# noway/nzcb-circom

Hardware: AMD Instinct MI355X
Metric: PLONK proofs/sec for nzcp_live (~2^21 constraints) at 1/2/4/8 MI355X (higher is better)
Workload: dtype u32 limbs: BN254 Fr/Fq Montgomery, 8x32-bit and 9x29-bit (MSM, NTT twiddles, quotient); 1 GPU; nzcp_live fullProve: NZCPPubIdentity(1,351,0,4,2,4) witness on the GPU (600560 signals) + PLONK proof, n=2^21, nPublic=3, 2970 inputs; domain_size=2097152, n_public=3, n_constraints=1785813, n_vars=1782570, n_additions=1182010, proofs_per_gpu=140, total_proofs=140, parallelism=batch-shard x1 (no collective), proofs_in_flight_per_gpu=5

## Files before the change

nzcb-circom_amd/csrc/prover.h:

```cpp
#pragma once
#include <chrono>
#include <functional>
#include <memory>
#include <string>
#include <vector>

#include "engine.h"
#include "zkey.h"

namespace nzcb {

struct AddRec {
  uint32_t ai, bi, dst, pad;
  Fr ac, bc;
};

struct MsmShard {
  static constexpr int kSlots = 3;
  int device = 0;
  size_t lo = 0, hi = 0;
  size_t llo = 0, lhi = 0;
  MsmBaseTable table, ltable;
  std::unique_ptr<MsmScratch> sc[kSlots];
  DevBuf<Fr> scal[kSlots];
  hipStream_t st[kSlots] = {nullptr, nullptr, nullptr};
  ~MsmShard();
};

struct Prover {
  uint32_t n = 0, n4 = 0, nVars = 0, nPublic = 0, nAdditions = 0, nConstraints = 0, nWit = 0;
  int power = 0;
  Fr k1, k2, wn, w2;
  std::vector<uint32_t> add_level_start;
  bool transcript_public = true;
  std::function<void(const std::string&)> log;

  std::unique_ptr<Engine> eng;
  static constexpr int kSlots = 3;
  std::unique_ptr<MsmScratch> msc[kSlots];
  hipStream_t aux[kSlots] = {nullptr, nullptr, nullptr};
  hipEvent_t ready[kSlots] = {nullptr, nullptr, nullptr};
  bool slot_split[kSlots] = {false, false, false};
  bool slot_lag[kSlots] = {false, false, false};
  hipEvent_t side_ready = nullptr, side_done = nullptr, pows_done = nullptr;
  ~Prover();
  DevBuf<G1Affine> ptau;
  MsmBaseTable ptab;
  DevBuf<G1Affine> ltau;
  MsmBaseTable ltab;
  bool lcommit = false;
  DevBuf<Fr> qm, ql, qr, qo, qc;
  DevBuf<Fr> sigma;
  DevBuf<Fr> sig_h;
  DevBuf<Fr> q_h;
  DevBuf<Fr> w_h;
  DevBuf<Fr> lagrange;
  DevBuf<uint32_t> amap, bmap, cmap;
  DevBuf<AddRec> adds;
  DevBuf<Fr> root_lo, root_hi;
  DevBuf<Fr> x_lo;
  DevBuf<Fr> g_lo, g_hi, gi_lo, gi_hi;
  DevBuf<F29> g29, gi29;
  Fr zh_inv[4];
  DevBuf<Fr> cq, cs, cl;
  bool quot3 = false;
  DevBuf<Fr> cq3, cs3, cl3;
  DevBuf<F29> tw3, itw3;
  Fr d3[3];
  Fr sig_top[3][4];
  DevBuf<Fr> wit;
  DevBuf<Fr> wtns_in;
  DevBuf<Fr> A, B, C, Z;
  DevBuf<Fr> pol_a, pol_b, pol_c, pol_z;
  DevBuf<Fr> A4, B4, C4, Z4, T, Tz, t;
  DevBuf<Fr> pol_r, pol_wxi, pol_wxiw;
  DevBuf<Fr> blind;
  DevBuf<Fr> scan_tmp;
  DevBuf<Fr> lin_tab;
  size_t lin_qn = 0;
  Fr* lin_tile_pows(int k);
  std::vector<Fr> lin_host;
  DevBuf<Fr> eval_part;
  DevBuf<F29> eval_pw;
  DevBuf<uint32_t> flags;
  std::vector<Fr> host_part;
  DevBuf<uint32_t> ntt_scr2;
  Fr* top_host = nullptr;
  static constexpr int kMbFlags = 24, kMbTotals = 25, kMbEvals = 27, kMbEvalMax = 8;
  size_t mb_apub = 0, mb_pubw = 0, mb_words = 0;

  int lane_id = 0;
  int fault = 0;
  double tm[11] = {0};
  bool prof_gpu = false;
  std::vector<std::pair<hipEvent_t, hipEvent_t>> span_ev;
  std::vector<int> span_kind;
  size_t spans_used = 0;
  size_t span_begin(int kind, hipStream_t s);
  void span_end(size_t i, hipStream_t s);
  void span_totals(double* msm_ms, double* ntt_ms);

  Prover(const uint8_t* zkey, size_t len, int device);
  Prover(const Prover& primary, int lane);
  void set_msm_devices(const std::vector<int>& devices);
  std::vector<std::unique_ptr<MsmShard>> shards;
  size_t own_hi = 0, own_lhi = 0;
  nzcb_msm_send_fn split_send = nullptr;
  nzcb_msm_gather_fn split_gather = nullptr;
  void* split_user = nullptr;
  int split_world = 1;
  size_t split_own = 0, split_own_l = 0;
  void set_msm_split(int world, size_t own_points, size_t own_lagrange, nzcb_msm_send_fn send,
                     nzcb_msm_gather_fn gather, void* user);
  void prove(const uint8_t* witness, size_t n_witness, const uint8_t* blinding, uint8_t* proof_out,
             uint8_t* pub_out, bool witness_on_device = false);

 private:
  hipStream_t st() const { return eng->stream; }
  void init_slots();
  void alloc_workspace();
  void to4t(const Fr* evals, Fr* coefs, Fr* evals4, const int* bidx, int nb, hipStream_t s = nullptr);
  void to4t_coefs(const Fr* evals, Fr* coefs, const int* bidx, int nb, hipStream_t s, uint32_t* scr = nullptr);
  void to4t_evals4(const Fr* coefs, Fr* evals4, int nb, hipStream_t s, uint32_t* scr = nullptr);
  void round3_quot3(const Fr& beta, const Fr& gamma, const Fr& alpha, hipStream_t s);
  void launch_gate_check(hipStream_t s);
  void copy_tops(hipStream_t s);
  void commit_start(int slot, const Fr* scalars, size_t len, const MsmBaseTable* tab = nullptr,
// ... 14 lines not shown
```

nzcb-circom_amd/csrc/prover.hip:

```cpp
#include <rocprofiler-sdk-roctx/roctx.h>
#include "lagrange.h"
#include "prover.h"
#include "transcript.h"

#include <cstring>
#include <cerrno>
#include <string>
#include <sys/random.h>

#include "keccak.h"

namespace nzcb {

static constexpr int kT = 256;
static constexpr uint32_t kZeroRef = 0xffffffffu;

__global__ void k_wit_to_mont(const Fr* __restrict__ in, Fr* __restrict__ out, size_t n) {
  size_t i = (size_t)blockIdx.x * blockDim.x + threadIdx.x;
  if (i >= n) return;
  out[i] = (i == 0) ? Fr::zero() : to_mont(in[i]);
}

__global__ void k_additions(const AddRec* __restrict__ recs, uint32_t count, Fr* __restrict__ wit) {
  uint32_t i = blockIdx.x * blockDim.x + threadIdx.x;
// ... 445 lines not shown
  for (int T = t1 - 1; T >= t0; T--) {
    suf = suf + h[T] * Q[T];
    h[T] = suf * Qinv[T];
  }
  if (tid == 0) h[m] = Fr::zero();
}

__global__ void k_stride4(const Fr* __restrict__ src, size_t n, Fr* __restrict__ dst) {
  const size_t i = (size_t)blockIdx.x * blockDim.x + threadIdx.x;
  if (i < n) dst[i] = src[4 * i];
}

struct QArgs {
  Fr beta, gamma, alpha, alpha2, bk1, bk2;
  Fr zhinv[4];
};

__global__ void __launch_bounds__(kT)
k_quotient_coset(const Fr* __restrict__ A, const Fr* __restrict__ B, const Fr* __restrict__ C,
                 const Fr* __restrict__ Z, const Fr* __restrict__ cq, const Fr* __restrict__ cs,
                 const Fr* __restrict__ cl, uint32_t npub, const Fr* __restrict__ Apub, size_t n,
                 const Fr* __restrict__ xlo, const Fr* __restrict__ xhi, QArgs q, Fr* __restrict__ T) {
  const size_t n4 = 4 * n;
  size_t i = (size_t)blockIdx.x * blockDim.x + threadIdx.x;
  if (i >= n4) return;
  const Fr a = A[i], b = B[i], c = C[i];
  const Fr x = xlo[i & 4095] * xhi[i >> 12];
  Fr gate = a * b * cq[i] + a * cq[n4 + i] + b * cq[2 * n4 + i] + c * cq[3 * n4 + i] + cq[4 * n4 + i];
  for (uint32_t j = 0; j < npub; j++) gate = gate - cl[j * n4 + i] * Apub[j];
  const Fr z = Z[i];
  const Fr bx = q.beta * x;
  Fr num = (a + bx + q.gamma) * (b + q.bk1 * x + q.gamma);
  num = num * (c + q.bk2 * x + q.gamma) * z;
  Fr den = (a + q.beta * cs[i] + q.gamma) * (b + q.beta * cs[n4 + i] + q.gamma);
  den = den * (c + q.beta * cs[2 * n4 + i] + q.gamma) * Z[(i + 4) & (n4 - 1)];
  const Fr e4 = (z - Fr::one()) * cl[i] * q.alpha2;
  T[i] = (gate + q.alpha * (num - den) + e4) * q.zhinv[i & 3];
}

constexpr uint32_t kQ29MaxPub = 8;

static bool quot3_enabled() {
  static const bool on = [] {
    const char* e = std::getenv("NZCB_QUOT3");
    return !(e && e[0] == '0');
  }();
  return on;
}
struct QArgs29 {
  F29 beta, bk1, bk2, alpha2, zhinv[4];
  F29 gamma, negone;
  int k23;
  F29 alpha;
};

template <int K>
__device__ __forceinline__ F29 q29_pi_chunk(const Fr* __restrict__ cl, const Fr* __restrict__ Apub, uint32_t j0,
                                            size_t n4, size_t i) {
  F29 pa[K], pb[K];
#pragma unroll
  for (int k = 0; k < K; k++) {
    pa[k] = split29(cl[(size_t)(j0 + k) * n4 + i]);
    pb[k] = split29(neg(Apub[j0 + k]));
  }
  return mulsum29<Fr29, K>(pa, pb);
}

__device__ __forceinline__ F29 q29_pi(const Fr* __restrict__ cl, const Fr* __restrict__ Apub, uint32_t j0,
                                      uint32_t cnt, size_t n4, size_t i) {
  switch (cnt) {
    case 1: return q29_pi_chunk<1>(cl, Apub, j0, n4, i);
    case 2: return q29_pi_chunk<2>(cl, Apub, j0, n4, i);
    case 3: return q29_pi_chunk<3>(cl, Apub, j0, n4, i);
    default: return q29_pi_chunk<4>(cl, Apub, j0, n4, i);
  }
}

template <bool THREE>
__global__ void __launch_bounds__(kT) __attribute__((amdgpu_waves_per_eu(4, 8)))
k_quotient_coset29(const Fr* __restrict__ A, const Fr* __restrict__ B, const Fr* __restrict__ C,
                   const Fr* __restrict__ Z, const Fr* __restrict__ cq, const Fr* __restrict__ cs,
                   const Fr* __restrict__ cl, uint32_t npub, const Fr* __restrict__ Apub, size_t n,
                   const Fr* __restrict__ xlo, const Fr* __restrict__ xhi, QArgs29 q, Fr* __restrict__ T) {
  const size_t n4 = (THREE ? 3 : 4) * n;
  size_t i = (size_t)blockIdx.x * blockDim.x + threadIdx.x;
  if (i >= n4) return;
  size_t ix, izw;
  int cj;
  if (THREE) {
    const int lg = __ffsll((long long)n) - 1;
    const size_t j = i >> lg, m = i & (n - 1);
    ix = 4 * m + j;
    izw = j * n + ((m + 1) & (n - 1));
    cj = (int)j;
  } else {
    ix = i;
    izw = (i + 4) & (n4 - 1);
    cj = (int)(i & 3);
  }
  const F29 a = split29(A[i]), b = split29(B[i]), c = split29(C[i]), z = split29(Z[i]);
  F29 gate;
  {
    const F29 ga[4] = {mul29<Fr29>(a, b), a, b, c};
    const F29 gb[4] = {split29(cq[i]), split29(cq[n4 + i]), split29(cq[2 * n4 + i]), split29(cq[3 * n4 + i])};
    gate = add29(mulsum29<Fr29, 4>(ga, gb), split29(cq[4 * n4 + i]));
  }
  if (npub > 0) gate = add29(gate, q29_pi(cl, Apub, 0, npub < 4 ? npub : 4, n4, i));
  if (npub > 4) gate = add29(gate, q29_pi(cl, Apub, 4, npub - 4, n4, i));
  const F29 x = mul29<Fr29>(split29(xlo[ix & 4095]), split29(xhi[ix >> 12]));
  const F29 bx = mul29<Fr29>(q.beta, x);
  const F29 bx2 = q.k23 ? add29(bx, bx) : mul29<Fr29>(q.bk1, x);
  const F29 bx3 = q.k23 ? add29(bx2, bx) : mul29<Fr29>(q.bk2, x);
  const F29 f1 = add29(add29(a, bx), q.gamma);
  const F29 f2 = add29(add29(b, bx2), q.gamma);
  const F29 f3 = add29(add29(c, bx3), q.gamma);
  const F29 num = mul29<Fr29>(mul29<Fr29>(mul29<Fr29>(f1, f2), f3), z);
  const F29 g1 = add29(add29(a, mul29<Fr29>(q.beta, split29(cs[i]))), q.gamma);
  const F29 g2 = add29(add29(b, mul29<Fr29>(q.beta, split29(cs[n4 + i]))), q.gamma);
  const F29 g3 = add29(add29(c, mul29<Fr29>(q.beta, split29(cs[2 * n4 + i]))), q.gamma);
  const F29 den = mul29<Fr29>(mul29<Fr29>(mul29<Fr29>(g1, g2), g3), split29(Z[izw]));
  const F29 pa[2] = {q.alpha, q.alpha2};
  const F29 pb[2] = {sub29(num, den, Fr29::K2), mul29<Fr29>(add29(z, q.negone), split29(cl[i]))};
  const F29 S = add29(gate, mulsum29<Fr29, 2>(pa, pb));
  T[i] = join_fr29(mul29<Fr29>(S, q.zhinv[cj]));
}

__global__ void __launch_bounds__(kT)
k_gate_h(const Fr* __restrict__ A, const Fr* __restrict__ B, const Fr* __restrict__ C, const Fr* __restrict__ qh,
         size_t n, uint32_t npub, uint32_t* __restrict__ flags) {
  const size_t m = (size_t)blockIdx.x * blockDim.x + threadIdx.x;
  if (m >= n) return;
  const Fr a = A[m], b = B[m], c = C[m];
  Fr g = qh[m] * a * b + qh[n + m] * a + qh[2 * n + m] * b + qh[3 * n + m] * c + qh[4 * n + m];
  if (m < npub) g = g - a;
  if (!g.is_zero()) atomicOr(flags, 1u);
}

struct T3Args {
  Fr c0[6], c1[6], c2[6], q3[6];
  Fr i4, two_over_d, inv_d2;
};
__global__ void __launch_bounds__(kT)
k_t_combine(const Fr* __restrict__ V, size_t n, T3Args a, Fr* __restrict__ t) {
  const size_t k = (size_t)blockIdx.x * blockDim.x + threadIdx.x;
  if (k >= n) return;
  Fr v0 = V[k], v1 = V[n + k], v2 = V[2 * n + k];
  if (k < 6) {
    v0 = v0 - a.c0[k];
    v1 = v1 - a.c1[k];
    v2 = v2 - a.c2[k];
  }
  const Fr sm = v0 + v2, dl = v0 - v2, im = dl * a.i4, v12 = v1 + v1;
  t[k] = sm + v12 - im;
  t[n + k] = dl * a.two_over_d;
  t[2 * n + k] = (sm - v12 + im) * a.inv_d2;
  if (k < 6) t[3 * n + k] = a.q3[k];
}

__global__ void k_root_n(Fr* __restrict__ out, const Fr* __restrict__ rlo, const Fr* __restrict__ rhi, size_t n) {
  const size_t i = (size_t)blockIdx.x * blockDim.x + threadIdx.x;
  if (i < n) out[i] = root4(rlo, rhi, 4 * i);
}

__global__ void k_fault_bump(Fr* x) {
  if (threadIdx.x == 0) x[0] = x[0] + Fr::one();
}

__global__ void k_dbl_pow(Fr* __restrict__ x, size_t m, int e) {
  size_t i = (size_t)blockIdx.x * blockDim.x + threadIdx.x;
  if (i >= m) return;
  Fr v = x[i];
  for (int k = 0; k < e; k++) v = v + v;
  x[i] = v;
}

static F29 f29_exp(Fr v, int extra) {
  for (int k = 0; k < extra; k++) v = v + v;
  return split29(v);
}

static constexpr int kEvalMax = 8;
static constexpr int kEvalBits = 16;
struct EvalSet {
  const Fr* p[kEvalMax];
  uint64_t len[kEvalMax];
  Fr x[kEvalMax];
  Fr x4096[kEvalMax];
  F29 x29[kEvalMax];
// ... 39 lines not shown
}

template <int NP>
__global__ void __launch_bounds__(kT) k_eval_multi(EvalSet es, const F29* __restrict__ pw, const Fr* __restrict__ pw2,
                                                   Fr* __restrict__ partial, int nblocks) {
  static_assert(NP <= kEvalMax && kEvalMax <= 4 * (kT / 64), "one 16-lane group per point");
  __shared__ Fr sh[kT / 64];
  __shared__ Fr bpow[kEvalMax];
  __shared__ Fr bsum[kEvalMax];
  {
    const int l = (int)(threadIdx.x & 63), k = l & 15, j = 4 * (int)(threadIdx.x >> 6) + (l >> 4);
    Fr f = Fr::one();
    if (j < NP && k < es.nbits && ((blockIdx.x >> k) & 1u)) f = pw2[j * kEvalBits + k];
    for (int m = 8; m >= 1; m >>= 1) f = f * shfl_fr(f, l ^ m);
    if (j < NP && k == 0) bpow[j] = f;
  }
  const size_t s = (size_t)blockIdx.x * kT * kEvalChunk2 + threadIdx.x;
  F29 acc[NP];
#pragma unroll
  for (int j = 0; j < NP; j++)
#pragma unroll
    for (int l = 0; l < 9; l++) acc[j].v[l] = 0;
  for (int m = kEvalChunk2 - 1; m >= 0; m--) {
    const size_t i = s + (size_t)m * kT;
#pragma unroll
    for (int j = 0; j < NP; j++)
      if (i < es.len[j]) {
        const F29 t = mul29<Fr29>(acc[j], es.y29[j]), c = split29(es.p[j][i]);
#pragma unroll
        for (int l = 0; l < 9; l++) acc[j].v[l] = t.v[l] + c.v[l];
      }
  }
#pragma unroll
  for (int j = 0; j < NP; j++) {
    const Fr r = block_sum_fr(join_fr29(mul29<Fr29>(acc[j], pw[(size_t)j * kT + threadIdx.x])), sh);
    if (threadIdx.x == 0) bsum[j] = r;
  }
  if (threadIdx.x < NP) partial[(size_t)threadIdx.x * nblocks + blockIdx.x] = bsum[threadIdx.x] * bpow[threadIdx.x];
}

__global__ void __launch_bounds__(kT) k_eval_sum(const Fr* __restrict__ partial, int nblocks, Fr* __restrict__ out) {
  __shared__ Fr sh[kT / 64];
  const int j = blockIdx.x;
  Fr acc = Fr::zero();
  for (int b = (int)threadIdx.x; b < nblocks; b += kT) acc = acc + partial[(size_t)j * nblocks + b];
  const Fr r = block_sum_fr(acc, sh);
  if (threadIdx.x == 0) {
    host_put(out + j, r);
    host_put_done();
  }
}

struct RArgs {
  Fr coefz, coef_ab, ea, eb, ec, coefs3;
};

__global__ void k_pol_r(const Fr* __restrict__ pz, const Fr* __restrict__ qm, const Fr* __restrict__ ql,
                        const Fr* __restrict__ qr, const Fr* __restrict__ qo, const Fr* __restrict__ qc,
                        const Fr* __restrict__ s3, size_t n, RArgs r, Fr* __restrict__ out) {
  size_t i = (size_t)blockIdx.x * blockDim.x + threadIdx.x;
  if (i >= n + 3) return;
  Fr v = r.coefz * pz[i];
  if (i < n) {
    v = v + r.coef_ab * qm[i] + r.ea * ql[i] + r.eb * qr[i] + r.ec * qo[i] + qc[i];
    v = v - r.coefs3 * s3[i];
  }
  out[i] = v;
}

struct WArgs {
  Fr xim, xi2m, v[7], w0sub;
};

__global__ void k_pol_wxi(const Fr* __restrict__ t, const Fr* __restrict__ pr, const Fr* __restrict__ pa,
                          const Fr* __restrict__ pb, const Fr* __restrict__ pc, const Fr* __restrict__ s1,
                          const Fr* __restrict__ s2, size_t n, WArgs wa, Fr* __restrict__ out) {
  size_t i = (size_t)blockIdx.x * blockDim.x + threadIdx.x;
  if (i >= n + 6) return;
  Fr w = wa.xi2m * t[2 * n + i];
  if (i < n) w = w + wa.xim * t[n + i] + t[i];
  if (i < n + 3) w = w + wa.v[1] * pr[i];
  if (i < n + 2) w = w + wa.v[2] * pa[i] + wa.v[3] * pb[i] + wa.v[4] * pc[i];
  if (i < n) w = w + wa.v[5] * s1[i] + wa.v[6] * s2[i];
  if (i == 0) w = w - wa.w0sub;
  out[i] = w;
}

__global__ void k_div_check(const Fr* __restrict__ src, Fr p0_adjust, const Fr* __restrict__ q, Fr d,
                            uint32_t* flags, uint32_t bit, uint32_t* __restrict__ mb_flags) {
  if (threadIdx.x || blockIdx.x) return;
  Fr p0 = src[0] - p0_adjust;
  if (!(p0 + d * q[0]).is_zero()) atomicOr(flags, bit);
  host_put(mb_flags, *flags);
  host_put_done();
}

__global__ void k_root_table(Fr* __restrict__ out, Fr base, Fr scale, size_t count) {
  size_t i = (size_t)blockIdx.x * blockDim.x + threadIdx.x;
  if (i >= count) return;
  out[i] = scale * pow_u64(base, i);
}

__global__ void k_factor29_table(F29* __restrict__ out, const Fr* __restrict__ lo, const Fr* __restrict__ hi, Fr scale,
                                 size_t count) {
  size_t i = (size_t)blockIdx.x * blockDim.x + threadIdx.x;
  if (i >= count) return;
  Fr v = lo[i & 4095] * hi[i >> 12] * scale;
#pragma unroll
  for (int k = 0; k < 5; k++) v = v + v;
  out[i] = split29(v);
}

static std::string fr_dec(const Fr& m) {
  Fr x = from_mont(m);
  uint32_t v[8];
  std::memcpy(v, x.v, 32);
  std::string s;
  bool nz = true;
  while (nz) {
    uint64_t rem = 0;
    nz = false;
    for (int i = 7; i >= 0; i--) {
      uint64_t cur = (rem << 32) | v[i];
      v[i] = (uint32_t)(cur / 10);
      rem = cur % 10;
      if (v[i]) nz = true;
    }
    s.push_back((char)('0' + rem));
  }
  return std::string(s.rbegin(), s.rend());
}

static Fr fr_small(uint64_t k) {
  Fr x = Fr::zero();
  x.v[0] = (uint32_t)k;
  x.v[1] = (uint32_t)(k >> 32);
  return to_mont(x);
}
// ... 233 lines not shown
                         q_h.p + (size_t)k * n);
    NZ_HIP(hipGetLastError());
  }
  if (quot3) {
    const size_t nhi3 = (n + 4095) / 4096;
    tw3.alloc((size_t)3 * n);
    itw3.alloc((size_t)3 * n);
    const Fr inv4n = inverse(fr_small(n4));
    DevBuf<Fr> lo, hi;
    for (int j = 0; j < 3; j++) {
      const Fr cj = g * pow_u64(w4, (uint64_t)j), cji = inverse(cj);
      d3[j] = pow_u64(cj, n);
      table(lo, nlo, cj, one);
      table(hi, nhi3, pow_u64(cj, 4096), one);
      hipLaunchKernelGGL(k_factor29_table, dim3(grid_for(n, kT, 1u << 30)), dim3(kT), 0, s, tw3.p + (size_t)j * n,
                         lo.p, hi.p, one, (size_t)n);
      NZ_HIP(hipStreamSynchronize(s));
      table(lo, nlo, cji, one);
      table(hi, nhi3, pow_u64(cji, 4096), one);
      hipLaunchKernelGGL(k_factor29_table, dim3(grid_for(n, kT, 1u << 30)), dim3(kT), 0, s, itw3.p + (size_t)j * n,
                         lo.p, hi.p, inv4n, (size_t)n);
      NZ_HIP(hipGetLastError());
      NZ_HIP(hipStreamSynchronize(s));
    }
    for (int k = 0; k < 3; k++)
      NZ_HIP(hipMemcpy(sig_top[k], sigma.p + (size_t)k * 5 * n + (n - 4), 4 * sizeof(Fr), hipMemcpyDeviceToHost));
  }
  if (quot3) {
    const uint32_t nl = nPublic > 0 ? nPublic : 1;
    const size_t n3 = (size_t)3 * n;
    cq3.alloc(5 * n3);
    cs3.alloc(3 * n3);
    cl3.alloc(nl * n3);
    auto coset3 = [&](const Fr* coefs, Fr* out) {
      for (int j = 0; j < 3; j++) {
        NttIo io;
        io.in_len = n;
        io.in_f = tw3.p + (size_t)j * n;
        ntt(eng->ntt_tables, coefs, out + (size_t)j * n, power, false, s, nullptr, &io);
      }
    };
    const DevBuf<Fr>* qs[5] = {&qm, &ql, &qr, &qo, &qc};
    for (int k = 0; k < 5; k++) coset3(qs[k]->p, cq3.p + (size_t)k * n3);
    for (int k = 0; k < 3; k++) coset3(sigma.p + (size_t)k * 5 * n, cs3.p + (size_t)k * n3);
    for (uint32_t j = 0; j < nl; j++) coset3(lagrange.p + (size_t)j * 5 * n, cl3.p + (size_t)j * n3);
    NZ_HIP(hipGetLastError());
    auto scale = [&](Fr* p, size_t m, int e) {
      hipLaunchKernelGGL(k_dbl_pow, dim3(grid_for(m, kT, 1u << 30)), dim3(kT), 0, s, p, m, e);
    };
    scale(cq3.p, n3, 10);
    scale(cq3.p + n3, 3 * n3, 5);
    scale(cl3.p, (size_t)nl * n3, 5);
    scale(x_lo.p, nlo, 5);
    NZ_HIP(hipGetLastError());
  } else {
    const uint32_t nl = nPublic > 0 ? nPublic : 1;
    cq.alloc((size_t)5 * n4);
    cs.alloc((size_t)3 * n4);
    cl.alloc((size_t)nl * n4);
    auto coset_eval = [&](const Fr* coefs, Fr* out) {
      NttIo io;
      io.in_len = n;
      io.in_f = g29.p;
      ntt(eng->ntt_tables, coefs, out, power + 2, false, s, nullptr, &io);
    };
    const DevBuf<Fr>* qs[5] = {&qm, &ql, &qr, &qo, &qc};
    for (int k = 0; k < 5; k++) coset_eval(qs[k]->p, cq.p + (size_t)k * n4);
    for (int k = 0; k < 3; k++) coset_eval(sigma.p + (size_t)k * 5 * n, cs.p + (size_t)k * n4);
    for (uint32_t j = 0; j < nl; j++) coset_eval(lagrange.p + (size_t)j * 5 * n, cl.p + (size_t)j * n4);
    NZ_HIP(hipGetLastError());
    if (nPublic <= kQ29MaxPub) {
      auto scale = [&](Fr* p, size_t m, int e) {
        hipLaunchKernelGGL(k_dbl_pow, dim3(grid_for(m, kT, 1u << 30)), dim3(kT), 0, s, p, m, e);
      };
      scale(cq.p, n4, 10);
      scale(cq.p + n4, 3 * n4, 5);
      scale(cl.p, (size_t)nl * n4, 5);
      scale(x_lo.p, nlo, 5);
      NZ_HIP(hipGetLastError());
    }
  }
  NZ_HIP(hipStreamSynchronize(s));
}

void Prover::init_slots() {
  for (int i = 0; i < kSlots; i++) {
    msc[i].reset(new MsmScratch());
#ifdef NZCB_AB_GENERIC
    msc[i]->init((size_t)n + 6, true, i == 0 ? 3 : 1, true);
#else
    msc[i]->init((size_t)n + 6, true, i == 0 ? 3 : 1, false);
#endif
    NZ_HIP(hipStreamCreateWithFlags(&aux[i], hipStreamNonBlocking));
    NZ_HIP(hipEventCreateWithFlags(&ready[i], hipEventDisableTiming));
  }
  NZ_HIP(hipEventCreateWithFlags(&side_ready, hipEventDisableTiming));
  NZ_HIP(hipEventCreateWithFlags(&side_done, hipEventDisableTiming));
  NZ_HIP(hipEventCreateWithFlags(&pows_done, hipEventDisableTiming));
  mb_apub = kMbEvals + kMbEvalMax;
  mb_pubw = mb_apub + nPublic;
  mb_words = mb_pubw + nPublic;
  NZ_HIP(hipHostMalloc((void**)&top_host, mb_words * sizeof(Fr), hipHostMallocCoherent));
  std::memset((void*)top_host, 0, mb_words * sizeof(Fr));
}

void Prover::alloc_workspace() {
  wit.alloc(nVars ? nVars : 1);
  wtns_in.alloc(nWit ? nWit : 1);
  A.alloc(n + 2); B.alloc(n + 2); C.alloc(n + 2); Z.alloc(n);
  pol_a.alloc(n + 2); pol_b.alloc(n + 2); pol_c.alloc(n + 2); pol_z.alloc(n + 3);
  const size_t ne = quot3 ? (size_t)3 * n : n4;
  A4.alloc(ne); B4.alloc(ne); C4.alloc(ne); Z4.alloc(ne);
  T.alloc(ne); Tz.alloc(ne); t.alloc(quot3 ? ne + 6 : n4);
  pol_r.alloc(n + 3); pol_wxi.alloc(n + 6); pol_wxiw.alloc(n + 3);
  blind.alloc(13);
  scan_tmp.alloc(3 * ((size_t)n / kTileN + 2) + 64);
  lin_qn = (size_t)n / kTileN + 3;
  lin_tab.alloc(2 * sizeof(LinTab) / sizeof(Fr) + 4 * lin_qn);
  lin_host.resize(2 * sizeof(LinTab) / sizeof(Fr));
  size_t nblocks = ((size_t)3 * n + 6 + (size_t)kT * kEvalChunk2 - 1) / ((size_t)kT * kEvalChunk2) + 1;
  eval_part.alloc((size_t)kEvalMax * nblocks + kEvalMax);
  eval_pw.alloc((size_t)kEvalMax * kT + (kEvalMax * kEvalBits * sizeof(Fr) + sizeof(F29) - 1) / sizeof(F29));
  host_part.resize(std::max<size_t>(nblocks, kEvalMax));
  flags.p = (uint32_t*)(blind.p + 12);
  flags.n = 1;
  flags.owned = false;
  const int zlog = quot3 ? power : power + 2;
  if (zlog > 8) ntt_scr2.alloc((size_t)9 << zlog);
}

Prover::Prover(const Prover& pk, int lane) {
  GuardScope guards;
  lane_id = lane;
  n = pk.n; n4 = pk.n4; nVars = pk.nVars; nPublic = pk.nPublic; nAdditions = pk.nAdditions;
  nConstraints = pk.nConstraints; nWit = pk.nWit; power = pk.power;
  k1 = pk.k1; k2 = pk.k2; wn = pk.wn; w2 = pk.w2;
  add_level_start = pk.add_level_start;
  transcript_public = pk.transcript_public;
  for (int k = 0; k < 4; k++) zh_inv[k] = pk.zh_inv[k];
  NZ_HIP(hipSetDevice(pk.eng->device));
  eng.reset(new Engine(pk.eng->device, power + 2, 0));
  init_slots();
  ptau.alias(pk.ptau);
  ptab.q.alias(pk.ptab.q);
  ptab.n = pk.ptab.n; ptab.stride = pk.ptab.stride; ptab.c = pk.ptab.c; ptab.nw = pk.ptab.nw;
  ptab.mont_folded = pk.ptab.mont_folded;
  lcommit = pk.lcommit;
  ltau.alias(pk.ltau);
  ltab.q.alias(pk.ltab.q);
  ltab.n = pk.ltab.n; ltab.stride = pk.ltab.stride; ltab.c = pk.ltab.c; ltab.nw = pk.ltab.nw;
  ltab.sparse = pk.ltab.sparse;
  qm.alias(pk.qm); ql.alias(pk.ql); qr.alias(pk.qr); qo.alias(pk.qo); qc.alias(pk.qc);
  sigma.alias(pk.sigma); sig_h.alias(pk.sig_h); q_h.alias(pk.q_h); w_h.alias(pk.w_h); lagrange.alias(pk.lagrange);
  amap.alias(pk.amap); bmap.alias(pk.bmap); cmap.alias(pk.cmap); adds.alias(pk.adds);
  root_lo.alias(pk.root_lo); root_hi.alias(pk.root_hi); x_lo.alias(pk.x_lo);
  g_lo.alias(pk.g_lo); g_hi.alias(pk.g_hi); gi_lo.alias(pk.gi_lo); gi_hi.alias(pk.gi_hi);
  g29.alias(pk.g29); gi29.alias(pk.gi29);
  cq.alias(pk.cq); cs.alias(pk.cs); cl.alias(pk.cl);
  quot3 = pk.quot3;
  cq3.alias(pk.cq3); cs3.alias(pk.cs3); cl3.alias(pk.cl3);
  tw3.alias(pk.tw3); itw3.alias(pk.itw3);
  for (int j = 0; j < 3; j++) d3[j] = pk.d3[j];
  std::memcpy(sig_top, pk.sig_top, sizeof(sig_top));
  alloc_workspace();
}

void Prover::launch_gate_check(hipStream_t s) {
  hipLaunchKernelGGL(k_gate_h, dim3(grid_for(n, kT, 1u << 30)), dim3(kT), 0, s, A.p, B.p, C.p, q_h.p, (size_t)n,
                     nPublic, flags.p);
  NZ_HIP(hipGetLastError());
}

void Prover::copy_tops(hipStream_t s) {
  hipLaunchKernelGGL(k_tops, dim3(1), dim3(32), 0, s, pol_a.p, pol_b.p, pol_c.p, pol_z.p, (size_t)n,
                     (const uint32_t*)flags.p, top_host);
  NZ_HIP(hipGetLastError());
  NZ_HIP(hipStreamSynchronize(s));
  if (top_host[kMbFlags].v[0] & 1u) throw Error(NZCB_ERR_T_DIV, "T Polynomial is not divisible");
}

void Prover::round3_quot3(const Fr& beta, const Fr& gamma, const Fr& alpha, hipStream_t s) {
  const size_t n3 = (size_t)3 * n;
  const bool side = lcommit;
  if (side) copy_tops(s);
  QArgs29 q29;
  q29.beta = f29_exp(beta, 5);
  q29.k23 = k1 == fr_small(2) && k2 == fr_small(3) ? 1 : 0;
  q29.bk1 = f29_exp(beta * k1, 5);
  q29.bk2 = f29_exp(beta * k2, 5);
  q29.alpha2 = f29_exp(alpha * alpha, 5);
  for (int k = 0; k < 4; k++) q29.zhinv[k] = f29_exp(zh_inv[k], 5);
  q29.gamma = f29_exp(gamma, 0);
  q29.negone = f29_exp(neg(Fr::one()), 0);
  q29.alpha = f29_exp(alpha, 20);
  hipLaunchKernelGGL((k_quotient_coset29<true>), dim3(grid_for(n3, kT, 1u << 30)), dim3(kT), 0, s, A4.p, B4.p, C4.p,
                     Z4.p, cq3.p, cs3.p, cl3.p, nPublic, A.p, (size_t)n, x_lo.p, root_hi.p, q29, T.p);
  if (!side) launch_gate_check(s);
  for (int j = 0; j < 3; j++) {
    NttIo io;
    io.out_f = itw3.p + (size_t)j * n;
    io.out_f_has_scale = true;
    {
      const size_t sp = prof_gpu ? span_begin(1, s) : 0;
      ntt(eng->ntt_tables, T.p + (size_t)j * n, Tz.p + (size_t)j * n, power, true, s, nullptr, &io);
      if (prof_gpu) span_end(sp, s);
    }
  }
  NZ_HIP(hipGetLastError());
  if (!side) copy_tops(s);
  Fr top[4][6];
  std::memcpy(top, top_host, sizeof(top));
  Fr p1[4][6], p2[4][6];
  const Fr w = wn, wi = inverse(wn);
  const Fr wpow[6] = {w * w, w, Fr::one(), wi, wi * wi, wi * wi * wi};
  for (int u = 0; u < 6; u++) {
    for (int f3 = 0; f3 < 3; f3++) {
      p1[f3][u] = top[f3][5 - u];
      p2[f3][u] = top[f3][5 - u];
      if (u >= 2) p2[f3][u] = p2[f3][u] + beta * sig_top[f3][5 - u];
    }
    p1[3][u] = top[3][5 - u];
    p2[3][u] = top[3][5 - u] * wpow[u];
  }
  auto conv = [](const Fr (&x)[6], const Fr (&y)[6], Fr (&out)[6]) {
    for (int s2 = 0; s2 < 6; s2++) {
      Fr acc = Fr::zero();
      for (int u = 0; u <= s2; u++) acc = acc + x[u] * y[s2 - u];
      out[s2] = acc;
    }
  };
  Fr e1[6], e2[6], e3[6], h1[6], h2[6], h3[6];
  conv(p1[0], p1[1], e1);
  conv(e1, p1[2], e2);
  conv(e2, p1[3], e3);
  conv(p2[0], p2[1], h1);
  conv(h1, p2[2], h2);
  conv(h2, p2[3], h3);
  T3Args ta;
  const Fr D = d3[0], D3 = D * D * D, i4 = d3[1] * inverse(D), quarter = inverse(fr_small(4));
  for (int k = 0; k < 6; k++) {
    ta.q3[k] = alpha * (e3[5 - k] - h3[5 - k]);
    const Fr c = D3 * ta.q3[k] * quarter;
    ta.c0[k] = c;
    ta.c1[k] = neg(i4 * c);
    ta.c2[k] = neg(c);
  }
  ta.i4 = i4;
  ta.two_over_d = fr_small(2) * inverse(D);
  ta.inv_d2 = inverse(D * D);
// ... 455 lines not shown
    hipLaunchKernelGGL(k_perm_tile, dim3((unsigned)ntiles), dim3(kT), 0, s, A.p, B.p, C.p, sig_h.p, (size_t)n,
                       w_h.p, pa, Z.p, ntot, dtot);
    hipLaunchKernelGGL(k_perm_factors, dim3(1), dim3(1024), 0, s, (const Fr*)ntot, (const Fr*)dtot, (int)ntiles,
                       fac, top_host + kMbTotals);
    NZ_HIP(hipGetLastError());
    NZ_HIP(hipStreamSynchronize(s));
    const Fr tt[2] = {top_host[kMbTotals], top_host[kMbTotals + 1]};
    if (tt[0] != tt[1]) throw Error(NZCB_ERR_COPY, "Copy constraints does not match");
    hipLaunchKernelGGL(k_apply_tiles, dim3((unsigned)ntiles), dim3(kT), 0, s, Z.p, (size_t)n,
                       (const Fr*)fac, inverse(tt[1]));
    NZ_HIP(hipGetLastError());
    const int bz[3] = {9, 8, 7};
    to4t_coefs(Z.p, pol_z.p, bz, 3, s, ntt_scr2.p);
    lg("multiexp Z");
    commit_start(0, pol_z.p, n + 3);
    to4t_evals4(pol_z.p, Z4.p, 3, s, ntt_scr2.p);
    pZ = commit_finish(0);
  }
  tm[3] = ms_since(t2);

  ranges.next("round3: quotient t + commit T1, T2, T3");
  auto t3 = std::chrono::steady_clock::now();
  Fr alpha;
  {
    std::vector<uint8_t> tr(64);
    g1_uncompressed(pZ, tr.data());
    alpha = hash_to_fr(tr);
    lg("alpha: " + fr_dec(alpha));
  }
  {
    QArgs q;
    q.beta = beta;
    q.gamma = gamma;
    q.alpha = alpha;
    q.alpha2 = alpha * alpha;
    q.bk1 = beta * k1;
    q.bk2 = beta * k2;
    for (int k = 0; k < 4; k++) q.zhinv[k] = zh_inv[k];
    auto tq = std::chrono::steady_clock::now();
    NZ_HIP(hipStreamWaitEvent(s, side_done, 0));
    if (quot3) {
      round3_quot3(beta, gamma, alpha, s);
    } else if (nPublic <= kQ29MaxPub) {
      QArgs29 q29;
      q29.beta = f29_exp(beta, 5);
      q29.k23 = k1 == fr_small(2) && k2 == fr_small(3) ? 1 : 0;
      q29.bk1 = f29_exp(q.bk1, 5);
      q29.bk2 = f29_exp(q.bk2, 5);
      q29.alpha2 = f29_exp(q.alpha2, 5);
      for (int k = 0; k < 4; k++) q29.zhinv[k] = f29_exp(zh_inv[k], 5);
      q29.gamma = f29_exp(gamma, 0);
      q29.negone = f29_exp(neg(Fr::one()), 0);
      q29.alpha = f29_exp(alpha, 20);
      hipLaunchKernelGGL((k_quotient_coset29<false>), dim3(grid_for(n4, kT, 1u << 30)), dim3(kT), 0, s, A4.p, B4.p,
                         C4.p, Z4.p, cq.p, cs.p, cl.p, nPublic, A.p, (size_t)n, x_lo.p, root_hi.p, q29, T.p);
    } else {
      hipLaunchKernelGGL(k_quotient_coset, dim3(grid_for(n4, kT, 1u << 30)), dim3(kT), 0, s, A4.p, B4.p, C4.p,
                         Z4.p, cq.p, cs.p, cl.p, nPublic, A.p, (size_t)n, x_lo.p, root_hi.p, q, T.p);
    }
    NZ_HIP(hipGetLastError());
    if (!quot3) {
      NttIo io;
      io.out_f = gi29.p;
      io.out_f_has_scale = true;
      io.out_limit = (size_t)3 * n + 6;
      io.out_flags = flags.p;
      {
        const size_t sp = prof_gpu ? span_begin(1, s) : 0;
        ntt(eng->ntt_tables, T.p, t.p, power + 2, true, s, nullptr, &io);
        if (prof_gpu) span_end(sp, s);
      }
      NZ_HIP(hipGetLastError());
      uint32_t f = 0;
      NZ_HIP(hipMemcpyAsync(&f, flags.p, 4, hipMemcpyDeviceToHost, s));
      NZ_HIP(hipStreamSynchronize(s));
      if (f & 1u) throw Error(NZCB_ERR_T_DIV, "T Polynomial is not divisible");
    }
    ntt_ms += ms_since(tq);
    if (fault == NZCB_FAULT_QUOTIENT) {
      fault = 0;
      hipLaunchKernelGGL(k_fault_bump, dim3(1), dim3(64), 0, s, t.p + 1);
      NZ_HIP(hipGetLastError());
    }
    lg("multiexp T1");
    commit_start(0, t.p, n);
    lg("multiexp T2");
    commit_start(1, t.p + n, n);
    lg("multiexp T3");
    commit_start(2, t.p + 2 * (size_t)n, n + 6);
    pT1 = commit_finish(0);
    pT2 = commit_finish(1);
    pT3 = commit_finish(2);
  }
  tm[4] = ms_since(t3);

  ranges.next("round4: evaluations");
  auto t4 = std::chrono::steady_clock::now();
  Fr xi, ea, eb, ec, es1, es2, et, ezw, er, xim;
  {
    std::vector<uint8_t> tr(192);
    g1_uncompressed(pT1, tr.data());
    g1_uncompressed(pT2, tr.data() + 64);
    g1_uncompressed(pT3, tr.data() + 128);
    xi = hash_to_fr(tr);
    lg("xi: " + fr_dec(xi));
    {
      const Fr* polys[7] = {pol_a.p, pol_b.p, pol_c.p, sigma.p, sigma.p + 5 * (size_t)n, t.p, pol_z.p};
      const size_t lens[7] = {n + 2, n + 2, n + 2, n, n, 3 * (size_t)n + 6, n + 3};
      const Fr xs[7] = {xi, xi, xi, xi, xi, xi, xi * wn};
      Fr ev[7];
      eval_many(7, polys, lens, xs, ev, [&] {
        lin_tables(0, xi, aux[2]);
        lin_tables(1, xi * wn, aux[2]);
        NZ_HIP(hipEventRecord(pows_done, aux[2]));
      });
      NZ_HIP(hipStreamWaitEvent(s, pows_done, 0));
      ea = ev[0];
      eb = ev[1];
      ec = ev[2];
      es1 = ev[3];
      es2 = ev[4];
      et = ev[5];
      ezw = ev[6];
    }
    Fr coef_ab = ea * eb;
    Fr betaxi = beta * xi;
    Fr e2 = (ea + betaxi + gamma) * (eb + betaxi * k1 + gamma);
    e2 = e2 * (ec + betaxi * k2 + gamma) * alpha;
    Fr e3 = (ea + beta * es1 + gamma) * (eb + beta * es2 + gamma);
    e3 = e3 * beta * ezw * alpha;
    xim = xi;
    for (int i = 0; i < power; i++) xim = sqr(xim);
    Fr eval_l1 = (xim - Fr::one()) * inverse((xi - Fr::one()) * fr_small(n));
    Fr e4 = eval_l1 * (alpha * alpha);
    RArgs ra{e2 + e4, coef_ab, ea, eb, ec, e3};
    hipLaunchKernelGGL(k_pol_r, dim3(grid_for(n + 3, kT, 1u << 30)), dim3(kT), 0, s, pol_z.p, qm.p, ql.p, qr.p,
                       qo.p, qc.p, sigma.p + 10 * (size_t)n, (size_t)n, ra, pol_r.p);
    NZ_HIP(hipGetLastError());
    {
      const Fr* polys[1] = {pol_r.p};
      const size_t lens[1] = {n + 3};
      eval_many(1, polys, lens, &xi, &er);
    }
    {
      const Fr zh = xim - Fr::one(), nf = fr_small(n);
      Fr pi = Fr::zero(), wj = Fr::one();
      for (uint32_t j = 0; j < nPublic; j++) {
        pi = pi - Apub[j] * wj * zh * inverse(nf * (xi - wj));
        wj = wj * wn;
      }
      const Fr perm = alpha * (ea + beta * es1 + gamma) * (eb + beta * es2 + gamma) * (ec + gamma) * ezw;
      if (et * zh != er + pi - perm - e4)
        throw Error(NZCB_ERR_INTERNAL, "quotient check failed: t(xi) Z_H(xi) differs from the numerator at xi");
    }
  }
  tm[5] = ms_since(t4);

  ranges.next("round5: Wxi, Wxiw + commit");
  auto t5 = std::chrono::steady_clock::now();
  {
    std::vector<uint8_t> tr(7 * 32);
    const Fr* ev[7] = {&ea, &eb, &ec, &es1, &es2, &ezw, &er};
    for (int i = 0; i < 7; i++) fr_to_be(*ev[i], tr.data() + 32 * i);
    WArgs wa;
    wa.v[0] = Fr::zero();
    wa.v[1] = hash_to_fr(tr);
    lg("v: " + fr_dec(wa.v[1]));
    for (int i = 2; i <= 6; i++) wa.v[i] = wa.v[i - 1] * wa.v[1];
    wa.xim = xim;
    wa.xi2m = xim * xim;
    wa.w0sub = et + wa.v[1] * er + wa.v[2] * ea + wa.v[3] * eb + wa.v[4] * ec + wa.v[5] * es1 + wa.v[6] * es2;
    hipLaunchKernelGGL(k_pol_wxi, dim3(grid_for(n + 6, kT, 1u << 30)), dim3(kT), 0, s, t.p, pol_r.p, pol_a.p,
                       pol_b.p, pol_c.p, sigma.p, sigma.p + 5 * (size_t)n, (size_t)n, wa, T.p);
    NZ_HIP(hipGetLastError());
    div_pol1(T.p, n + 6, 0, Fr::zero(), pol_wxi.p, 4u);
    lg("multiexp Wxi");
    commit_start(0, pol_wxi.p, n + 6);
    div_pol1(pol_z.p, n + 3, 1, ezw, pol_wxiw.p, 4u);
    lg("multiexp Wxiw");
    commit_start(1, pol_wxiw.p, n + 3);
    NZ_HIP(hipStreamSynchronize(s));
    const uint32_t f = top_host[kMbFlags].v[0];
    pWxi = commit_finish(0);
    pWxiw = commit_finish(1);
    if (f & 4u) throw Error(NZCB_ERR_DIVPOL, "Polinomial does not divide");
  }
  tm[6] = ms_since(t5);
  tm[0] = ms_since(T0);
  tm[7] = msm_ms;
  tm[8] = ntt_ms;
  tm[9] = tm[10] = -1;
  if (prof_gpu) span_totals(&tm[9], &tm[10]);

  const G1Affine* pts[9] = {&pA, &pB, &pC, &pZ, &pT1, &pT2, &pT3, &pWxi, &pWxiw};
  for (int i = 0; i < 9; i++) {
    uint8_t* o = proof_out + 64 * i;
    if (pts[i]->is_inf()) {
      std::memset(o, 0, 64);
    } else {
      Fq x = from_mont(pts[i]->x), y = from_mont(pts[i]->y);
      std::memcpy(o, x.v, 32);
      std::memcpy(o + 32, y.v, 32);
    }
  }
  const Fr* ev[7] = {&ea, &eb, &ec, &es1, &es2, &ezw, &er};
  for (int i = 0; i < 7; i++) fr_to_le_normal(*ev[i], proof_out + 9 * 64 + 32 * i);
  for (uint32_t i = 0; i < nPublic; i++) {
    fr_to_le_normal(top_host[mb_pubw + i], pub_out + 32 * (size_t)i);
  }
}

}
```

Before: 47.49 proofs/s.

## Port pol_r, pol_wxi and gate check to 29-bit limbs; fold coset scaling

Rewrites k_pol_r, k_pol_wxi and the gate check kernel to use the 9x29-bit lazy-reduction arithmetic with mulsum dot products instead of serial 8x32 Montgomery ops. In the 3-coset quotient path it precomputes beta*x_hi per block and folds the per-coset Z_H inverse into the selector and Lagrange tables and into alpha. This removes one multiply per element in the quotient kernel and the final zhinv multiply. It adds setup-time table rescaling and depends on the lazy-reduction exponent bounds in f29_exp being correct.

```diff
diff --git a/nzcb-circom_amd/csrc/prover.h b/nzcb-circom_amd/csrc/prover.h
--- a/nzcb-circom_amd/csrc/prover.h
+++ b/nzcb-circom_amd/csrc/prover.h
@@ -73,6 +73,7 @@
   DevBuf<Fr> A, B, C, Z;
   DevBuf<Fr> pol_a, pol_b, pol_c, pol_z;
   DevBuf<Fr> A4, B4, C4, Z4, T, Tz, t;
+  DevBuf<Fr> bx_hi;
   DevBuf<Fr> pol_r, pol_wxi, pol_wxiw;
   DevBuf<Fr> blind;
   DevBuf<Fr> scan_tmp;
diff --git a/nzcb-circom_amd/csrc/prover.hip b/nzcb-circom_amd/csrc/prover.hip
--- a/nzcb-circom_amd/csrc/prover.hip
+++ b/nzcb-circom_amd/csrc/prover.hip
@@ -521,7 +521,22 @@
   F29 gamma, negone;
   int k23;
   F29 alpha;
+  F29 alphaz[3];
 };
+
+__global__ void k_beta_xhi(const Fr* __restrict__ xhi, Fr beta, size_t count, Fr* __restrict__ bxhi) {
+  const size_t k = (size_t)blockIdx.x * blockDim.x + threadIdx.x;
+  if (k < count) bxhi[k] = beta * xhi[k];
+}
+
+struct Z3Args {
+  Fr z[3];
+};
+__global__ void k_scale_coset3(Fr* __restrict__ p, size_t n, size_t arrays, Z3Args za) {
+  const size_t i = (size_t)blockIdx.x * blockDim.x + threadIdx.x;
+  if (i >= arrays * 3 * n) return;
+  p[i] = p[i] * za.z[(i / n) % 3];
+}
 
 template <int K>
 __device__ __forceinline__ F29 q29_pi_chunk(const Fr* __restrict__ cl, const Fr* __restrict__ Apub, uint32_t j0,
@@ -550,7 +565,8 @@
 k_quotient_coset29(const Fr* __restrict__ A, const Fr* __restrict__ B, const Fr* __restrict__ C,
                    const Fr* __restrict__ Z, const Fr* __restrict__ cq, const Fr* __restrict__ cs,
                    const Fr* __restrict__ cl, uint32_t npub, const Fr* __restrict__ Apub, size_t n,
-                   const Fr* __restrict__ xlo, const Fr* __restrict__ xhi, QArgs29 q, Fr* __restrict__ T) {
+                   const Fr* __restrict__ xlo, const Fr* __restrict__ xhi, const Fr* __restrict__ bxhi, QArgs29 q,
+                   Fr* __restrict__ T) {
   const size_t n4 = (THREE ? 3 : 4) * n;
   size_t i = (size_t)blockIdx.x * blockDim.x + threadIdx.x;
   if (i >= n4) return;
@@ -576,10 +592,17 @@
   }
   if (npub > 0) gate = add29(gate, q29_pi(cl, Apub, 0, npub < 4 ? npub : 4, n4, i));
   if (npub > 4) gate = add29(gate, q29_pi(cl, Apub, 4, npub - 4, n4, i));
-  const F29 x = mul29<Fr29>(split29(xlo[ix & 4095]), split29(xhi[ix >> 12]));
-  const F29 bx = mul29<Fr29>(q.beta, x);
-  const F29 bx2 = q.k23 ? add29(bx, bx) : mul29<Fr29>(q.bk1, x);
-  const F29 bx3 = q.k23 ? add29(bx2, bx) : mul29<Fr29>(q.bk2, x);
+  F29 bx, bx2, bx3;
+  if (THREE && q.k23) {
+    bx = mul29<Fr29>(split29(bxhi[ix >> 12]), split29(xlo[ix & 4095]));
+    bx2 = add29(bx, bx);
+    bx3 = add29(bx2, bx);
+  } else {
+    const F29 x = mul29<Fr29>(split29(xlo[ix & 4095]), split29(xhi[ix >> 12]));
+    bx = mul29<Fr29>(q.beta, x);
+    bx2 = q.k23 ? add29(bx, bx) : mul29<Fr29>(q.bk1, x);
+    bx3 = q.k23 ? add29(bx2, bx) : mul29<Fr29>(q.bk2, x);
+  }
   const F29 f1 = add29(add29(a, bx), q.gamma);
   const F29 f2 = add29(add29(b, bx2), q.gamma);
   const F29 f3 = add29(add29(c, bx3), q.gamma);
@@ -588,10 +611,13 @@
   const F29 g2 = add29(add29(b, mul29<Fr29>(q.beta, split29(cs[n4 + i]))), q.gamma);
   const F29 g3 = add29(add29(c, mul29<Fr29>(q.beta, split29(cs[2 * n4 + i]))), q.gamma);
   const F29 den = mul29<Fr29>(mul29<Fr29>(mul29<Fr29>(g1, g2), g3), split29(Z[izw]));
-  const F29 pa[2] = {q.alpha, q.alpha2};
+  const F29 pa[2] = {THREE ? q.alphaz[cj] : q.alpha, q.alpha2};
   const F29 pb[2] = {sub29(num, den, Fr29::K2), mul29<Fr29>(add29(z, q.negone), split29(cl[i]))};
   const F29 S = add29(gate, mulsum29<Fr29, 2>(pa, pb));
-  T[i] = join_fr29(mul29<Fr29>(S, q.zhinv[cj]));
+  if constexpr (THREE)
+    T[i] = canon_fr29(S);
+  else
+    T[i] = join_fr29(mul29<Fr29>(S, q.zhinv[cj]));
 }
 
 __global__ void __launch_bounds__(kT)
@@ -599,10 +625,12 @@
          size_t n, uint32_t npub, uint32_t* __restrict__ flags) {
   const size_t m = (size_t)blockIdx.x * blockDim.x + threadIdx.x;
   if (m >= n) return;
-  const Fr a = A[m], b = B[m], c = C[m];
-  Fr g = qh[m] * a * b + qh[n + m] * a + qh[2 * n + m] * b + qh[3 * n + m] * c + qh[4 * n + m];
-  if (m < npub) g = g - a;
-  if (!g.is_zero()) atomicOr(flags, 1u);
+  const F29 a = split29(A[m]), b = split29(B[m]), c = split29(C[m]);
+  const F29 ga[4] = {mul29<Fr29>(a, b), a, b, c};
+  const F29 gb[4] = {split29(qh[m]), split29(qh[n + m]), split29(qh[2 * n + m]), split29(qh[3 * n + m])};
+  F29 g = add29(mulsum29<Fr29, 4>(ga, gb), split29(qh[4 * n + m]));
+  if (m < npub) g = sub29(g, a, Fr29::K2);
+  if (!canon_fr29(g).is_zero()) atomicOr(flags, 1u);
 }
 
 struct T3Args {
@@ -748,38 +776,56 @@
 }
 
 struct RArgs {
-  Fr coefz, coef_ab, ea, eb, ec, coefs3;
+  F29 coefz, coef_ab, ea, eb, ec, ncoefs3;
 };
 
-__global__ void k_pol_r(const Fr* __restrict__ pz, const Fr* __restrict__ qm, const Fr* __restrict__ ql,
-                        const Fr* __restrict__ qr, const Fr* __restrict__ qo, const Fr* __restrict__ qc,
-                        const Fr* __restrict__ s3, size_t n, RArgs r, Fr* __restrict__ out) {
+__global__ void __launch_bounds__(kT)
+k_pol_r(const Fr* __restrict__ pz, const Fr* __restrict__ qm, const Fr* __restrict__ ql,
+        const Fr* __restrict__ qr, const Fr* __restrict__ qo, const Fr* __restrict__ qc,
+        const Fr* __restrict__ s3, size_t n, RArgs r, Fr* __restrict__ out) {
   size_t i = (size_t)blockIdx.x * blockDim.x + threadIdx.x;
   if (i >= n + 3) return;
-  Fr v = r.coefz * pz[i];
+  F29 v;
   if (i < n) {
-    v = v + r.coef_ab * qm[i] + r.ea * ql[i] + r.eb * qr[i] + r.ec * qo[i] + qc[i];
-    v = v - r.coefs3 * s3[i];
-  }
-  out[i] = v;
+    const F29 sa[6] = {r.coefz, r.coef_ab, r.ea, r.eb, r.ec, r.ncoefs3};
+    const F29 sb[6] = {split29(pz[i]), split29(qm[i]), split29(ql[i]),
+                       split29(qr[i]), split29(qo[i]), split29(s3[i])};
+    v = add29(mulsum29<Fr29, 6>(sa, sb), split29(qc[i]));
+  } else {
+    v = mul29<Fr29>(r.coefz, split29(pz[i]));
+  }
+  out[i] = canon_fr29(v);
 }
 
 struct WArgs {
-  Fr xim, xi2m, v[7], w0sub;
+  F29 xim, xi2m, v[7], nw0sub;
 };
 
-__global__ void k_pol_wxi(const Fr* __restrict__ t, const Fr* __restrict__ pr, const Fr* __restrict__ pa,
-                          const Fr* __restrict__ pb, const Fr* __restrict__ pc, const Fr* __restrict__ s1,
-                          const Fr* __restrict__ s2, size_t n, WArgs wa, Fr* __restrict__ out) {
+__global__ void __launch_bounds__(kT)
+k_pol_wxi(const Fr* __restrict__ t, const Fr* __restrict__ pr, const Fr* __restrict__ pa,
+          const Fr* __restrict__ pb, const Fr* __restrict__ pc, const Fr* __restrict__ s1,
+          const Fr* __restrict__ s2, size_t n, WArgs wa, Fr* __restrict__ out) {
   size_t i = (size_t)blockIdx.x * blockDim.x + threadIdx.x;
   if (i >= n + 6) return;
-  Fr w = wa.xi2m * t[2 * n + i];
-  if (i < n) w = w + wa.xim * t[n + i] + t[i];
-  if (i < n + 3) w = w + wa.v[1] * pr[i];
-  if (i < n + 2) w = w + wa.v[2] * pa[i] + wa.v[3] * pb[i] + wa.v[4] * pc[i];
-  if (i < n) w = w + wa.v[5] * s1[i] + wa.v[6] * s2[i];
-  if (i == 0) w = w - wa.w0sub;
-  out[i] = w;
+  F29 w;
+  if (i < n) {
+    const F29 sa[6] = {wa.xi2m, wa.xim, wa.v[1], wa.v[2], wa.v[3], wa.v[4]};
+    const F29 sb[6] = {split29(t[2 * n + i]), split29(t[n + i]), split29(pr[i]),
+                       split29(pa[i]), split29(pb[i]), split29(pc[i])};
+    const F29 ta[2] = {wa.v[5], wa.v[6]};
+    const F29 tb[2] = {split29(s1[i]), split29(s2[i])};
+    w = add3_29(mulsum29<Fr29, 6>(sa, sb), mulsum29<Fr29, 2>(ta, tb), split29(t[i]));
+    if (i == 0) w = add29(w, wa.nw0sub);
+  } else {
+    w = mul29<Fr29>(wa.xi2m, split29(t[2 * n + i]));
+    if (i < n + 3) w = add29(w, mul29<Fr29>(wa.v[1], split29(pr[i])));
+    if (i < n + 2) {
+      const F29 sa[3] = {wa.v[2], wa.v[3], wa.v[4]};
+      const F29 sb[3] = {split29(pa[i]), split29(pb[i]), split29(pc[i])};
+      w = add29(w, mulsum29<Fr29, 3>(sa, sb));
+    }
+  }
+  out[i] = canon_fr29(w);
 }
 
 __global__ void k_div_check(const Fr* __restrict__ src, Fr p0_adjust, const Fr* __restrict__ q, Fr d,
@@ -1119,6 +1165,13 @@
     scale(cq3.p + n3, 3 * n3, 5);
     scale(cl3.p, (size_t)nl * n3, 5);
     scale(x_lo.p, nlo, 5);
+    const Z3Args za{{zh_inv[0], zh_inv[1], zh_inv[2]}};
+    hipLaunchKernelGGL(k_scale_coset3, dim3(grid_for(5 * n3, kT, 1u << 30)), dim3(kT), 0, s, cq3.p, (size_t)n,
+                       (size_t)5, za);
+    hipLaunchKernelGGL(k_scale_coset3, dim3(grid_for((size_t)nl * n3, kT, 1u << 30)), dim3(kT), 0, s, cl3.p,
+                       (size_t)n, (size_t)nl, za);
+    scale(q_h.p, n, 10);
+    scale(q_h.p + n, 3 * (size_t)n, 5);
     NZ_HIP(hipGetLastError());
   } else {
     const uint32_t nl = nPublic > 0 ? nPublic : 1;
@@ -1179,6 +1232,7 @@
   const size_t ne = quot3 ? (size_t)3 * n : n4;
   A4.alloc(ne); B4.alloc(ne); C4.alloc(ne); Z4.alloc(ne);
   T.alloc(ne); Tz.alloc(ne); t.alloc(quot3 ? ne + 6 : n4);
+  if (quot3) bx_hi.alloc((n4 + 4095) / 4096);
   pol_r.alloc(n + 3); pol_wxi.alloc(n + 6); pol_wxiw.alloc(n + 3);
   blind.alloc(13);
   scan_tmp.alloc(3 * ((size_t)n / kTileN + 2) + 64);
@@ -1260,8 +1314,11 @@
   q29.gamma = f29_exp(gamma, 0);
   q29.negone = f29_exp(neg(Fr::one()), 0);
   q29.alpha = f29_exp(alpha, 20);
+  for (int j = 0; j < 3; j++) q29.alphaz[j] = f29_exp(alpha * zh_inv[j], 20);
+  const size_t nhi = (n4 + 4095) / 4096;
+  hipLaunchKernelGGL(k_beta_xhi, dim3(grid_for(nhi, kT)), dim3(kT), 0, s, root_hi.p, beta, nhi, bx_hi.p);
   hipLaunchKernelGGL((k_quotient_coset29<true>), dim3(grid_for(n3, kT, 1u << 30)), dim3(kT), 0, s, A4.p, B4.p, C4.p,
-                     Z4.p, cq3.p, cs3.p, cl3.p, nPublic, A.p, (size_t)n, x_lo.p, root_hi.p, q29, T.p);
+                     Z4.p, cq3.p, cs3.p, cl3.p, nPublic, A.p, (size_t)n, x_lo.p, root_hi.p, bx_hi.p, q29, T.p);
   if (!side) launch_gate_check(s);
   for (int j = 0; j < 3; j++) {
     NttIo io;
@@ -1823,8 +1880,10 @@
       q29.gamma = f29_exp(gamma, 0);
       q29.negone = f29_exp(neg(Fr::one()), 0);
       q29.alpha = f29_exp(alpha, 20);
+      for (int j = 0; j < 3; j++) q29.alphaz[j] = q29.alpha;
       hipLaunchKernelGGL((k_quotient_coset29<false>), dim3(grid_for(n4, kT, 1u << 30)), dim3(kT), 0, s, A4.p, B4.p,
-                         C4.p, Z4.p, cq.p, cs.p, cl.p, nPublic, A.p, (size_t)n, x_lo.p, root_hi.p, q29, T.p);
+                         C4.p, Z4.p, cq.p, cs.p, cl.p, nPublic, A.p, (size_t)n, x_lo.p, root_hi.p,
+                         (const Fr*)nullptr, q29, T.p);
     } else {
       hipLaunchKernelGGL(k_quotient_coset, dim3(grid_for(n4, kT, 1u << 30)), dim3(kT), 0, s, A4.p, B4.p, C4.p,
                          Z4.p, cq.p, cs.p, cl.p, nPublic, A.p, (size_t)n, x_lo.p, root_hi.p, q, T.p);
@@ -1904,7 +1963,8 @@
     for (int i = 0; i < power; i++) xim = sqr(xim);
     Fr eval_l1 = (xim - Fr::one()) * inverse((xi - Fr::one()) * fr_small(n));
     Fr e4 = eval_l1 * (alpha * alpha);
-    RArgs ra{e2 + e4, coef_ab, ea, eb, ec, e3};
+    RArgs ra{f29_exp(e2 + e4, 5), f29_exp(coef_ab, 5), f29_exp(ea, 5),
+             f29_exp(eb, 5),      f29_exp(ec, 5),      f29_exp(neg(e3), 5)};
     hipLaunchKernelGGL(k_pol_r, dim3(grid_for(n + 3, kT, 1u << 30)), dim3(kT), 0, s, pol_z.p, qm.p, ql.p, qr.p,
                        qo.p, qc.p, sigma.p + 10 * (size_t)n, (size_t)n, ra, pol_r.p);
     NZ_HIP(hipGetLastError());
@@ -1933,14 +1993,16 @@
     std::vector<uint8_t> tr(7 * 32);
     const Fr* ev[7] = {&ea, &eb, &ec, &es1, &es2, &ezw, &er};
     for (int i = 0; i < 7; i++) fr_to_be(*ev[i], tr.data() + 32 * i);
+    Fr v[7];
+    v[0] = Fr::zero();
+    v[1] = hash_to_fr(tr);
+    lg("v: " + fr_dec(v[1]));
+    for (int i = 2; i <= 6; i++) v[i] = v[i - 1] * v[1];
     WArgs wa;
-    wa.v[0] = Fr::zero();
-    wa.v[1] = hash_to_fr(tr);
-    lg("v: " + fr_dec(wa.v[1]));
-    for (int i = 2; i <= 6; i++) wa.v[i] = wa.v[i - 1] * wa.v[1];
-    wa.xim = xim;
-    wa.xi2m = xim * xim;
-    wa.w0sub = et + wa.v[1] * er + wa.v[2] * ea + wa.v[3] * eb + wa.v[4] * ec + wa.v[5] * es1 + wa.v[6] * es2;
+    for (int i = 0; i <= 6; i++) wa.v[i] = f29_exp(v[i], 5);
+    wa.xim = f29_exp(xim, 5);
+    wa.xi2m = f29_exp(xim * xim, 5);
+    wa.nw0sub = f29_exp(neg(et + v[1] * er + v[2] * ea + v[3] * eb + v[4] * ec + v[5] * es1 + v[6] * es2), 0);
     hipLaunchKernelGGL(k_pol_wxi, dim3(grid_for(n + 6, kT, 1u << 30)), dim3(kT), 0, s, t.p, pol_r.p, pol_a.p,
                        pol_b.p, pol_c.p, sigma.p, sigma.p + 5 * (size_t)n, (size_t)n, wa, T.p);
     NZ_HIP(hipGetLastError());
```

New measurement: 47.79 proofs/s (median of 6 runs). No clear change (+0.6%).
